# sharc-lab/FlowGNN

Measured on AMD Instinct MI355X. Metric: graphs/sec on ogbg-molhiv (GIN, dim=100), higher is better.
Workload: dtype f32; 1 GPU; GIN dim=100, batched ogbg-molhiv-shaped graphs on MI355X (BASELINE configs[1]); graphs_rank0=262144, nodes_rank0=6707949, edges_rank0=14754960, parallelism=single GPU

## Files before the change

### flowgnn_amd/csrc/dev/gin_pp_device.inc

```
constexpr int PP_ROWS = 128, PP_EDGES = 640;
constexpr int PP_PIECE = 14336, PP_PIECES = 14;
constexpr int PP_HDR_OFF = 13440;
constexpr int PP_TBL_STRIDE = 52;
constexpr int PP_TBL_BYTES = EDGE_COMBOS * PP_TBL_STRIDE * 4;
constexpr int PP_DESC_RP = PP_EDGES * 2;
constexpr int PP_DESC_PERM = PP_DESC_RP + 272;
constexpr int PP_DESC_BYTES = 1792;
constexpr int PP_SUB = 7;

__global__ __launch_bounds__(128) void gin_pp_prep_kernel(const int* __restrict__ row_ptr, const int* __restrict__ src,
                                                          const uint8_t* __restrict__ ecode, const int4* __restrict__ tiles,
                                                          uint8_t* __restrict__ desc, int n_tiles, int ntc) {
    constexpr int NKEY = 18;
    __shared__ int s_cnt[2][NKEY];
    const int tile = blockIdx.x;
    if (tile >= n_tiles) return;
    const int4 t = tiles[tile];
    const int t0 = t.x;
    int rows = t.y;
    if (rows > PP_ROWS) rows = PP_ROWS;
    const int e0 = row_ptr[t0];
    int ne = row_ptr[t0 + rows] - e0;
    if (ne > PP_EDGES) ne = PP_EDGES;
    uint8_t* d = desc + (size_t)tile * PP_DESC_BYTES;
// ... 29 lines not shown
        }
    const int pos = below + mine;
    const int kt = pos >> 4, j = pos & 15;
    if (ntc == 1) {
        d[PP_DESC_PERM + pos] = (uint8_t)r;
        return;
    }
    const int w4 = kt < 4 ? kt : 7 - kt, nt = kt < 4 ? 0 : 1;
    d[PP_DESC_PERM + w4 * 32 + nt * 16 + j] = (uint8_t)r;
}

#define PP_LD(off) (*reinterpret_cast<const uint4_t*>(wb + (off) + lane * 16))
template <bool PACKED, int NTC>
__device__ __forceinline__ void pp_w2(const char* wb, int lane, const uint4_t (&hb_hi)[NTC], const uint4_t (&hb_lo)[NTC], float4_t (&acc2)[NTC][GS_T2]) {
    if constexpr (PACKED) {
        uint4_t p[GS_T2];
#pragma unroll
        for (int t = 0; t < GS_T2; t++) p[t] = PP_LD(t * 1024);
#pragma unroll
        for (int t = 0; t < GS_T2; t++) {
            acc2[0][t] = GS_MFMA16(p[t], hb_hi[0], acc2[0][t]);
            if constexpr (NTC == 2) acc2[NTC - 1][t] = GS_MFMA16(p[t], hb_hi[NTC - 1], acc2[NTC - 1][t]);
        }
    } else {
        uint4_t f0[2], f1[2];
#define PP_U2_LOAD(F, T) F[0] = PP_LD((2 * (T)) * 1024); F[1] = PP_LD((2 * (T) + 1) * 1024);
#define PP_U2_MFMA(F, T)                                                                                    \
    acc2[0][T] = GS_MFMA16(F[0], hb_hi[0], acc2[0][T]);                                                     \
    if constexpr (NTC == 2) acc2[NTC - 1][T] = GS_MFMA16(F[0], hb_hi[NTC - 1], acc2[NTC - 1][T]);           \
    acc2[0][T] = GS_MFMA16(F[0], hb_lo[0], acc2[0][T]);                                                     \
    if constexpr (NTC == 2) acc2[NTC - 1][T] = GS_MFMA16(F[0], hb_lo[NTC - 1], acc2[NTC - 1][T]);           \
    acc2[0][T] = GS_MFMA16(F[1], hb_hi[0], acc2[0][T]);                                                     \
    if constexpr (NTC == 2) acc2[NTC - 1][T] = GS_MFMA16(F[1], hb_hi[NTC - 1], acc2[NTC - 1][T]);
        PP_U2_LOAD(f0, 0) GR_SB();
        PP_U2_LOAD(f1, 1) GR_SB(); PP_U2_MFMA(f0, 0) GR_SB();
        PP_U2_LOAD(f0, 2) GR_SB(); PP_U2_MFMA(f1, 1) GR_SB();
        PP_U2_LOAD(f1, 3) GR_SB(); PP_U2_MFMA(f0, 2) GR_SB();
        PP_U2_LOAD(f0, 4) GR_SB(); PP_U2_MFMA(f1, 3) GR_SB();
        PP_U2_LOAD(f1, 5) GR_SB(); PP_U2_MFMA(f0, 4) GR_SB();
        PP_U2_LOAD(f0, 6) GR_SB(); PP_U2_MFMA(f1, 5) GR_SB();
        PP_U2_MFMA(f0, 6) GR_SB();
#undef PP_U2_LOAD
#undef PP_U2_MFMA
    }
}

template <int NTL, bool DOT, int NTC>
__device__ __forceinline__ void pp_w1(const char* wb, int lane, int g, const uint4_t (&in_hi)[NTC][3], const uint4_t (&in_lo)[NTC][3],
                                      const uint4_t (&in_tb)[NTC], uint4_t (&hb_hi)[NTC], uint4_t (&hb_lo)[NTC], float& vmax,
                                      const float* u_step, float (&dot)[NTC]) {
    uint4_t f0[2], f1[2];
    float4_t acc1[NTC];
#define PP_U1_LOAD(F, TL, KS) F[0] = PP_LD((TL) * 6144 + (2 * (KS)) * 1024); F[1] = PP_LD((TL) * 6144 + (2 * (KS) + 1) * 1024);
#define PP_U1_MFMA1(F, KS)                                                                                  \
    acc1[0] = GS_MFMA16(F[0], in_hi[0][KS], acc1[0]);                                                       \
    if constexpr (NTC == 2) acc1[NTC - 1] = GS_MFMA16(F[0], in_hi[NTC - 1][KS], acc1[NTC - 1]);             \
    acc1[0] = GS_MFMA16(F[0], in_lo[0][KS], acc1[0]);                                                       \
    if constexpr (NTC == 2) acc1[NTC - 1] = GS_MFMA16(F[0], in_lo[NTC - 1][KS], acc1[NTC - 1]);             \
    acc1[0] = GS_MFMA16(F[1], in_hi[0][KS], acc1[0]);                                                       \
    if constexpr (NTC == 2) acc1[NTC - 1] = GS_MFMA16(F[1], in_hi[NTC - 1][KS], acc1[NTC - 1]);
#define PP_TAIL_LOAD(F, TL) F[0] = *reinterpret_cast<const uint4_t*>(wb + GRC_TAIL_OFF + (TL) * 512 + (lane & 31) * 16);
#define PP_BIAS(TL) acc1[0] = *reinterpret_cast<const float4_t*>(wb + GRC_B1_OFF + (TL) * 64 + g * 16);
#define PP_FINISH(TL)                                                                                     \
    _Pragma("unroll") for (int nt = 0; nt < NTC; nt++) {                                                    \
        float4_t r = acc1[nt];                                                                            \
        r.x = gs_relu(r.x); r.y = gs_relu(r.y); r.z = gs_relu(r.z); r.w = gs_relu(r.w);                   \
        if constexpr (DOT) {                                                                              \
            const float4 uu = *reinterpret_cast<const float4*>(u_step + 16 * (TL) + 4 * g);              \
            dot[nt] += r.x * uu.x; dot[nt] += r.y * uu.y; dot[nt] += r.z * uu.z; dot[nt] += r.w * uu.w;   \
            continue;                                                                                     \
        }                                                                                                 \
        vmax = __builtin_fmaxf(__builtin_fmaxf(vmax, r.x), r.y);                                          \
        vmax = __builtin_fmaxf(__builtin_fmaxf(vmax, r.z), r.w);                                          \
        if ((TL) == 0) { GS_SPLIT2(r.x, r.y, hb_hi[nt].x, hb_lo[nt].x); GS_SPLIT2(r.z, r.w, hb_hi[nt].y, hb_lo[nt].y); } \
        else { GS_SPLIT2(r.x, r.y, hb_hi[nt].z, hb_lo[nt].z); GS_SPLIT2(r.z, r.w, hb_hi[nt].w, hb_lo[nt].w); }           \
    }
    PP_U1_LOAD(f1, 0, 0)
    PP_BIAS(0)
    GR_SB();
    if constexpr (NTC == 2) acc1[NTC - 1] = acc1[0];
    PP_U1_LOAD(f0, 0, 1) GR_SB(); PP_U1_MFMA1(f1, 0) GR_SB();
    PP_U1_LOAD(f1, 0, 2) GR_SB(); PP_U1_MFMA1(f0, 1) GR_SB();
    PP_TAIL_LOAD(f0, 0) GR_SB(); PP_U1_MFMA1(f1, 2) GR_SB();
    if constexpr (NTL == 2) { PP_U1_LOAD(f1, 1, 0) GR_SB(); }
    acc1[0] = GS_MFMA16(f0[0], in_tb[0], acc1[0]);
    if constexpr (NTC == 2) acc1[NTC - 1] = GS_MFMA16(f0[0], in_tb[NTC - 1], acc1[NTC - 1]);
    if constexpr (NTL == 2) {
        PP_FINISH(0)
        PP_BIAS(1)
        if constexpr (NTC == 2) acc1[NTC - 1] = acc1[0];
        PP_U1_LOAD(f0, 1, 1) GR_SB(); PP_U1_MFMA1(f1, 0) GR_SB();
        PP_U1_LOAD(f1, 1, 2) GR_SB(); PP_U1_MFMA1(f0, 1) GR_SB();
        PP_TAIL_LOAD(f0, 1) GR_SB(); PP_U1_MFMA1(f1, 2) GR_SB();
        acc1[0] = GS_MFMA16(f0[0], in_tb[0], acc1[0]);
        if constexpr (NTC == 2) acc1[NTC - 1] = GS_MFMA16(f0[0], in_tb[NTC - 1], acc1[NTC - 1]);
        PP_FINISH(1)
    } else if constexpr (DOT) {
        PP_FINISH(0)
    } else {
        PP_FINISH(0)
#pragma unroll
        for (int nt = 0; nt < NTC; nt++) {
            const uint32_t ox = __shfl(hb_hi[nt].x, lane & 31, 64), oy = __shfl(hb_hi[nt].y, lane & 31, 64);
            const bool own = g < 2;
            hb_hi[nt] = own ? (uint4_t){hb_hi[nt].x, hb_hi[nt].y, hb_lo[nt].x, hb_lo[nt].y} : (uint4_t){ox, oy, 0u, 0u};
        }
    }
    asm volatile("" : "+v"(vmax));
#undef PP_U1_LOAD
#undef PP_U1_MFMA1
#undef PP_TAIL_LOAD
#undef PP_BIAS
#undef PP_FINISH
}
#undef PP_LD

__device__ __forceinline__ void pp_dma(const void* gsrc, void* ldst, int bytes, int wi, int nw, int lane) {
    const int pieces = (bytes + 1023) >> 10;
    const uint32_t lb = lds_addr_of(ldst);
    for (int pc = wi; pc < pieces; pc += nw) {
        const int left = bytes - pc * 1024;
        if (left >= 1024 || lane * 16 < left) lds_dma16(reinterpret_cast<const char*>(gsrc) + (size_t)pc * 1024, (uint32_t)lane * 16u, lb + pc * 1024);
    }
}
__device__ __forceinline__ void pp_dma_slice(const void* gsrc, void* ldst, int bytes, int first, int count, int wi, int nw, int lane) {
    const int pieces = (bytes + 1023) >> 10;
    const uint32_t lb = lds_addr_of(ldst);
    for (int pc = first + wi; pc < first + count && pc < pieces; pc += nw) {
        const int left = bytes - pc * 1024;
        if (left >= 1024 || lane * 16 < left) lds_dma16(reinterpret_cast<const char*>(gsrc) + (size_t)pc * 1024, (uint32_t)lane * 16u, lb + pc * 1024);
    }
}

// ... 340 lines not shown
```

### flowgnn_amd/csrc/gin_split.hip

```cpp
#include "gin_split.h"

#include <cmath>
#include <cstring>
#include <cstdlib>
#include <cstdio>
#include <vector>

#include "device_common.h"

#ifndef GS_SINGLE_PRODUCT
#define GS_SINGLE_PRODUCT 0
#endif
#ifndef GS_POOL_TU
#define GS_POOL_TU 0
#endif
#ifndef GS_NLOGIT_TU
#define GS_NLOGIT_TU 0
#endif
#ifndef GS_POOLSUM_TU
#define GS_POOLSUM_TU 0
#endif
#ifndef GS_POOL_MAX
#define GS_POOL_MAX 0
#endif
// ... 53 lines not shown
    } while (0)

typedef _Float16 half2_t __attribute__((ext_vector_type(2)));
__device__ __forceinline__ uint32_t gs_pack_rne(float a, float b) { return __builtin_bit_cast(uint32_t, (half2_t){(_Float16)a, (_Float16)b}); }
__device__ __forceinline__ float gs_rne(float a) { return (float)(_Float16)a; }
#define GS_OPER2(F16_, a, b, HI, LO)                                              \
    do {                                                                          \
        if constexpr (F16_) { (HI) = gs_pack_rne((a), (b)); (LO) = 0u; }          \
        else { GS_SPLIT2(a, b, HI, LO); }                                         \
    } while (0)

__device__ __forceinline__ float gs_relu(float x) {
    const int b = __builtin_bit_cast(int, x);
    return __builtin_bit_cast(float, b > 0 ? b : 0);
}

constexpr int GS_HUB = 8;
constexpr int GS_MAXHUB = 4;
template <int CTRL>
__device__ __forceinline__ float gs_dpp(float v) {
    return __builtin_bit_cast(float, __builtin_amdgcn_update_dpp(0, __builtin_bit_cast(int, v), CTRL, 0xF, 0xF, true));
}

template <int WAVES>
__device__ __forceinline__ void gs_issue_chunk(const uint8_t* __restrict__ gchunk, char* lds_buf, int wave, int lane) {
#pragma unroll
    for (int p = 0; p < (27 + WAVES - 1) / WAVES; p++) {
        const int piece = wave + WAVES * p;
        if (piece < 26 || (piece == 26 && lane < 40)) {
            const uint8_t* g = gchunk + piece * 1024 + lane * 16;
            __builtin_amdgcn_global_load_lds((const __attribute__((address_space(1))) void*)g,
                                             (__attribute__((address_space(3))) void*)(lds_buf + piece * 1024), 16, 0, 0);
        }
    }
}

template <int NT, bool F16>
__device__ __forceinline__ void gs_step(const char* wb, int s, int lane, int g, const uint4_t (&in_hi)[NT][3],
                                        const uint4_t (&in_lo)[NT][3], const float (&in_t)[NT], uint4_t (&h_hi)[NT],
                                        uint4_t (&h_lo)[NT], float4_t (&acc2)[NT][GS_T2], float& vmax) {
    uint4_t n_hi[NT], n_lo[NT];
    if (s < GS_STEPS - 1) {
        float4_t acc1[2][NT];
#pragma unroll
        for (int tl = 0; tl < 2; tl++) {
            const float4 b = *reinterpret_cast<const float4*>(wb + GS_B1_OFF + tl * 64 + g * 16);
#pragma unroll
            for (int nt = 0; nt < NT; nt++) acc1[tl][nt] = (float4_t){b.x, b.y, b.z, b.w};
        }
#pragma unroll
        for (int ks = 0; ks < 3; ks++) {
            uint4_t a[2][2];
#pragma unroll
            for (int tl = 0; tl < 2; tl++)
#pragma unroll
                for (int p = 0; p < (F16 ? 1 : 2); p++)
                    a[tl][p] = *reinterpret_cast<const uint4_t*>(wb + ((ks * 2 + tl) * 2 + p) * 1024 + lane * 16);
#pragma unroll
            for (int tl = 0; tl < 2; tl++)
#pragma unroll
                for (int nt = 0; nt < NT; nt++) acc1[tl][nt] = GS_MFMA16(a[tl][0], in_hi[nt][ks], acc1[tl][nt]);
            if constexpr (!F16) {
#pragma unroll
                for (int tl = 0; tl < 2; tl++)
#pragma unroll
                    for (int nt = 0; nt < NT; nt++) acc1[tl][nt] = GS_MFMA16(a[tl][0], in_lo[nt][ks], acc1[tl][nt]);
#pragma unroll
                for (int tl = 0; tl < 2; tl++)
#pragma unroll
                    for (int nt = 0; nt < NT; nt++) acc1[tl][nt] = GS_MFMA16(a[tl][1], in_hi[nt][ks], acc1[tl][nt]);
            }
        }
#pragma unroll
        for (int tl = 0; tl < 2; tl++) {
            const float at = *reinterpret_cast<const float*>(wb + GS_TAIL_OFF + tl * 256 + lane * 4);
#pragma unroll
            for (int nt = 0; nt < NT; nt++) acc1[tl][nt] = GS_MFMA32(at, in_t[nt], acc1[tl][nt]);
        }
#pragma unroll
        for (int nt = 0; nt < NT; nt++) {
            float4_t r0 = acc1[0][nt], r1 = acc1[1][nt];
            r0.x = gs_relu(r0.x); r0.y = gs_relu(r0.y); r0.z = gs_relu(r0.z); r0.w = gs_relu(r0.w);
            r1.x = gs_relu(r1.x); r1.y = gs_relu(r1.y); r1.z = gs_relu(r1.z); r1.w = gs_relu(r1.w);
            vmax = __builtin_fmaxf(__builtin_fmaxf(vmax, r0.x), r0.y);
            vmax = __builtin_fmaxf(__builtin_fmaxf(vmax, r0.z), r0.w);
            vmax = __builtin_fmaxf(__builtin_fmaxf(vmax, r1.x), r1.y);
            vmax = __builtin_fmaxf(__builtin_fmaxf(vmax, r1.z), r1.w);
            asm volatile("" : "+v"(vmax));
            GS_OPER2(F16, r0.x, r0.y, n_hi[nt].x, n_lo[nt].x);
            GS_OPER2(F16, r0.z, r0.w, n_hi[nt].y, n_lo[nt].y);
            GS_OPER2(F16, r1.x, r1.y, n_hi[nt].z, n_lo[nt].z);
            GS_OPER2(F16, r1.z, r1.w, n_hi[nt].w, n_lo[nt].w);
        }
    }
    if (s > 0) {
#pragma unroll
        for (int t0 = 0; t0 < GS_T2; t0 += 2) {
            uint4_t a[2][2];
#pragma unroll
            for (int tl = 0; tl < 2; tl++)
#pragma unroll
                for (int p = 0; p < (F16 ? 1 : 2); p++)
                    if (t0 + tl < GS_T2)
                        a[tl][p] = *reinterpret_cast<const uint4_t*>(wb + GS_W2_OFF + ((t0 + tl) * 2 + p) * 1024 + lane * 16);
#pragma unroll
            for (int tl = 0; tl < 2; tl++)
#pragma unroll
                for (int nt = 0; nt < NT; nt++)
                    if (t0 + tl < GS_T2) acc2[nt][t0 + tl] = GS_MFMA16(a[tl][0], h_hi[nt], acc2[nt][t0 + tl]);
            if constexpr (!F16) {
#pragma unroll
                for (int tl = 0; tl < 2; tl++)
#pragma unroll
                    for (int nt = 0; nt < NT; nt++)
                        if (t0 + tl < GS_T2) acc2[nt][t0 + tl] = GS_MFMA16(a[tl][0], h_lo[nt], acc2[nt][t0 + tl]);
#pragma unroll
                for (int tl = 0; tl < 2; tl++)
#pragma unroll
                    for (int nt = 0; nt < NT; nt++)
                        if (t0 + tl < GS_T2) acc2[nt][t0 + tl] = GS_MFMA16(a[tl][1], h_hi[nt], acc2[nt][t0 + tl]);
            }
        }
    }
    if (s < GS_STEPS - 1) {
#pragma unroll
        for (int nt = 0; nt < NT; nt++) { h_hi[nt] = n_hi[nt]; h_lo[nt] = n_lo[nt]; }
    }
}

#if GS_EPS
template <int NT, int WAVES, bool F16>
#else
template <int NT, int WAVES>
#endif
__global__ __launch_bounds__(WAVES * 64) void gin_layer_split_kernel(const float* __restrict__ h, float* __restrict__ hout,
                                                               const int* __restrict__ row_ptr,
                                                               const int* __restrict__ src,
                                                               const uint8_t* __restrict__ ecode,
                                                               const float* __restrict__ ecomb,
                                                               const uint8_t* __restrict__ wchunks, int n_tot, int relu_out,
                                                               int* __restrict__ range_flag, const float* __restrict__ pool_w
#if GS_EPS
                                                               , float self_s
// ... 231 lines not shown
                float4_t r = acc2[nt][t2] * oscale;
                if (relu_out) { r.x = gs_relu(r.x); r.y = gs_relu(r.y); r.z = gs_relu(r.z); r.w = gs_relu(r.w); }
                *reinterpret_cast<float4*>(row + col) = make_float4(r.x, r.y, r.z, r.w);
            }
        }
    }
    }
    if (__any(!(vmax < 6.0e4f))) {
        if (lane == 0) atomicOr(range_flag, 1);
    }
}

constexpr int GR_ROWS = 256;
constexpr int GR_EDGES = 1280;
constexpr float GR_MSG_SCALE = 1.0f / 65536.0f, GR_MSG_UNSCALE = 65536.0f;
constexpr int GR_WAVES = 8;
constexpr int GR_STEPS = 7;

constexpr int GRC_PK_OFF = 6144;
constexpr int GRC_PK6_OFF = 12288 + 512;
constexpr int GRC_TAIL_OFF = 12288;
constexpr int GRC_B1_OFF = 13312;
constexpr int GRC_W2_OFF = 13440;
constexpr int GRC_CHUNK_BYTES = 27776;
constexpr int GRC_CHUNK_STRIDE = 28672;

#ifndef GR_DEALERS
#define GR_DEALERS 4
#endif
#ifndef GR_DEAL_BASE
#define GR_DEAL_BASE 0
#endif
template <int DEAL>
__device__ __forceinline__ int gr_dealer(int wave) {
    if (DEAL >= GR_WAVES) return wave;
    const int d = wave - GR_DEAL_BASE;
    return (d >= 0 && d < DEAL) ? d : -1;
}
template <int DEAL = GR_DEALERS>
__device__ __forceinline__ void grc_issue_chunk(const uint8_t* __restrict__ gchunk, char* lds_buf, int wave, int lane) {
    wave = gr_dealer<DEAL>(wave);
    if (wave < 0) return;
    const uint32_t lb = lds_addr_of(lds_buf);
#pragma unroll
    for (int p = 0; p < (28 + DEAL - 1) / DEAL; p++) {
        const int piece = wave + DEAL * p;
        if (piece < 27 || (piece == 27 && lane < 8)) lds_dma16(gchunk + piece * 1024, (uint32_t)lane * 16u, lb + piece * 1024);
    }
}

template <int DEAL = GR_DEALERS>
__device__ __forceinline__ void grc_issue_chunk_w1(const uint8_t* __restrict__ gchunk, char* lds_buf, int wave, int lane) {
    wave = gr_dealer<DEAL>(wave);
    if (wave < 0) return;
    const uint32_t lb = lds_addr_of(lds_buf);
#pragma unroll
    for (int p = 0; p < (14 + DEAL - 1) / DEAL; p++) {
        const int piece = wave + DEAL * p;
        if (piece < 13 || (piece == 13 && lane < 8)) lds_dma16(gchunk + piece * 1024, (uint32_t)lane * 16u, lb + piece * 1024);
    }
}

#define GR_LD(off) (*reinterpret_cast<const uint4_t*>(wb + (off) + lane * 16))
#define GR_SB() __builtin_amdgcn_sched_barrier(0)
#ifndef GR_DEFER
#define GR_DEFER false
#endif
#ifndef GR_PRIO_HALF
#define GR_PRIO_HALF true
#endif
// ... 14 lines not shown
#define GR_PRIO_BY_PHASE true
#endif

struct GrNoHook { __device__ __forceinline__ void operator()() const {} };
template <int KIND, bool F16, bool PEND_IN = false, bool PEND_OUT = false, class HOOK = GrNoHook>
__device__ __forceinline__ void gr_step(const char* wb, int lane, int g, const uint4_t (&in_hi)[2][3], const uint4_t (&in_lo)[2][3],
                                        const uint4_t (&in_tb)[2], uint4_t (&hb_hi)[2], uint4_t (&hb_lo)[2], float4_t (&acc2)[2][GS_T2],
                                        float& vmax, float4_t (&pend)[2], const float* u_step = nullptr, float* dot = nullptr, int wave = 0,
                                        HOOK hook = HOOK()) {
    static_assert(KIND == 0 || KIND == 1 || KIND == 4 || KIND == 5, "step kinds");
    constexpr bool DO2 = KIND == 1, DO1 = true, DOT = KIND >= 4;
#define GR_PRIO_FLIP(TO_OLD) if (GR_FLIP) { if ((wave >= 4) != (TO_OLD)) __builtin_amdgcn_s_setprio(1); else __builtin_amdgcn_s_setprio(0); }
    constexpr int NTL = KIND == 5 ? 1 : 2;
    uint4_t f0[2], f1[2];
#define GR_U2_LOAD(F, T) F[0] = GR_LD(GRC_W2_OFF + (2 * (T)) * 1024); if constexpr (!F16) F[1] = GR_LD(GRC_W2_OFF + (2 * (T) + 1) * 1024);
#define GR_U2_MFMA(F, T)                                              \
    acc2[0][T] = GS_MFMA16(F[0], hb_hi[0], acc2[0][T]);               \
    acc2[1][T] = GS_MFMA16(F[0], hb_hi[1], acc2[1][T]);               \
    if constexpr (!F16) {                                             \
        acc2[0][T] = GS_MFMA16(F[0], hb_lo[0], acc2[0][T]);           \
        acc2[1][T] = GS_MFMA16(F[0], hb_lo[1], acc2[1][T]);           \
        acc2[0][T] = GS_MFMA16(F[1], hb_hi[0], acc2[0][T]);           \
        acc2[1][T] = GS_MFMA16(F[1], hb_hi[1], acc2[1][T]);           \
    }
#define GR_U1_LOAD(F, TL, KS) F[0] = GR_LD((TL) * 6144 + (2 * (KS)) * 1024); if constexpr (!F16) F[1] = GR_LD((TL) * 6144 + (2 * (KS) + 1) * 1024);
    float4_t acc1[2];
#define GR_U1_MFMA1(F, KS)                                            \
    acc1[0] = GS_MFMA16(F[0], in_hi[0][KS], acc1[0]);                 \
    acc1[1] = GS_MFMA16(F[0], in_hi[1][KS], acc1[1]);                 \
    if constexpr (!F16) {                                             \
        acc1[0] = GS_MFMA16(F[0], in_lo[0][KS], acc1[0]);             \
        acc1[1] = GS_MFMA16(F[0], in_lo[1][KS], acc1[1]);             \
        acc1[0] = GS_MFMA16(F[1], in_hi[0][KS], acc1[0]);             \
        acc1[1] = GS_MFMA16(F[1], in_hi[1][KS], acc1[1]);             \
    }
#define GR_TAIL_LOAD(F, TL) F[0] = *reinterpret_cast<const uint4_t*>(wb + GRC_TAIL_OFF + (TL) * 512 + (lane & 31) * 16);
#define GR_BIAS(TL) acc1[0] = *reinterpret_cast<const float4_t*>(wb + GRC_B1_OFF + (TL) * 64 + g * 16);
#define GR_FINISH(TL) GR_FINISH_FROM(acc1, TL)
#define GR_FINISH_FROM(SRC, TL)                                                                           \
    _Pragma("unroll") for (int nt = 0; nt < 2; nt++) {                                                    \
        float4_t r = SRC[nt];                                                                             \
        r.x = gs_relu(r.x); r.y = gs_relu(r.y); r.z = gs_relu(r.z); r.w = gs_relu(r.w);                   \
        if constexpr (DOT) {                                                                              \
            if constexpr (F16) {  \
                vmax = __builtin_fmaxf(__builtin_fmaxf(vmax, r.x), r.y);                                  \
                vmax = __builtin_fmaxf(__builtin_fmaxf(vmax, r.z), r.w);                                  \
                r.x = gs_rne(r.x); r.y = gs_rne(r.y); r.z = gs_rne(r.z); r.w = gs_rne(r.w);               \
            }                                                                                             \
            const float4 uu = *reinterpret_cast<const float4*>(u_step + 16 * (TL) + 4 * g);              \
            dot[nt] += r.x * uu.x; dot[nt] += r.y * uu.y; dot[nt] += r.z * uu.z; dot[nt] += r.w * uu.w;   \
            continue;                                                                                     \
        }                                                                                                 \
        vmax = __builtin_fmaxf(__builtin_fmaxf(vmax, r.x), r.y);                                          \
        vmax = __builtin_fmaxf(__builtin_fmaxf(vmax, r.z), r.w);                                          \
        if ((TL) == 0) { GS_OPER2(F16, r.x, r.y, hb_hi[nt].x, hb_lo[nt].x); GS_OPER2(F16, r.z, r.w, hb_hi[nt].y, hb_lo[nt].y); } \
        else { GS_OPER2(F16, r.x, r.y, hb_hi[nt].z, hb_lo[nt].z); GS_OPER2(F16, r.z, r.w, hb_hi[nt].w, hb_lo[nt].w); }           \
    }
    if constexpr (DO2) {
        GR_U2_LOAD(f0, 0)
        GR_SB();
        GR_U2_LOAD(f1, 1) GR_SB();
        if constexpr (PEND_IN) { GR_FINISH_FROM(pend, 1) GR_SB(); }
        GR_U2_MFMA(f0, 0) GR_SB();
        GR_U2_LOAD(f0, 2) GR_SB(); GR_U2_MFMA(f1, 1) GR_SB();
        GR_U2_LOAD(f1, 3) GR_SB(); GR_U2_MFMA(f0, 2) GR_SB();
        GR_U2_LOAD(f0, 4) GR_SB(); GR_U2_MFMA(f1, 3) GR_SB();
        GR_U2_LOAD(f1, 5) GR_SB(); GR_U2_MFMA(f0, 4) GR_SB();
        GR_U2_LOAD(f0, 6) GR_SB(); GR_U2_MFMA(f1, 5) GR_SB();
        GR_U1_LOAD(f1, 0, 0)
        GR_BIAS(0)
        GR_SB();
        GR_U2_MFMA(f0, 6)
        GR_SB();
        GR_PRIO_FLIP(true)
    }
    if constexpr (DO1) {
        if constexpr (!DO2) {
            GR_U1_LOAD(f1, 0, 0)
            GR_BIAS(0)
            GR_SB();
        }
        acc1[1] = acc1[0];
        GR_U1_LOAD(f0, 0, 1) GR_SB(); GR_U1_MFMA1(f1, 0) GR_SB();
        GR_U1_LOAD(f1, 0, 2) GR_SB(); GR_U1_MFMA1(f0, 1) GR_SB();
        GR_TAIL_LOAD(f0, 0) GR_SB(); GR_U1_MFMA1(f1, 2) GR_SB();
        if constexpr (NTL == 2) { GR_U1_LOAD(f1, 1, 0) GR_SB(); }
        acc1[0] = GS_MFMA16(f0[0], in_tb[0], acc1[0]);
        acc1[1] = GS_MFMA16(f0[0], in_tb[1], acc1[1]);
        if constexpr (NTL == 2) {
            if constexpr (!DO2) { GR_PRIO_FLIP(true) }
            GR_FINISH(0)
            GR_BIAS(1)
            if constexpr (DOT) { GR_SB(); hook(); GR_SB(); }
            acc1[1] = acc1[0];
            GR_U1_LOAD(f0, 1, 1) GR_SB(); GR_U1_MFMA1(f1, 0) GR_SB();
            GR_U1_LOAD(f1, 1, 2) GR_SB(); GR_U1_MFMA1(f0, 1) GR_SB();
            GR_TAIL_LOAD(f0, 1) GR_SB(); GR_U1_MFMA1(f1, 2) GR_SB();
            acc1[0] = GS_MFMA16(f0[0], in_tb[0], acc1[0]);
            acc1[1] = GS_MFMA16(f0[0], in_tb[1], acc1[1]);
            if constexpr (PEND_OUT) { pend[0] = acc1[0]; pend[1] = acc1[1]; }
            else { GR_FINISH(1) }
        } else {
            static_assert(DOT, "a one-tile step is the folded layer's last (KIND 5)");
            GR_SB(); hook(); GR_SB();
            GR_FINISH(0)
        }
        asm volatile("" : "+v"(vmax));
    }
    if constexpr (DO2 || NTL == 2) { GR_PRIO_FLIP(false) }
#undef GR_PRIO_FLIP
#undef GR_U1_MFMA1
#undef GR_TAIL_LOAD
#undef GR_BIAS
#undef GR_FINISH
#undef GR_FINISH_FROM
#undef GR_U2_LOAD
#undef GR_U2_MFMA
#undef GR_U1_LOAD
}
template <int STORE, bool F16>
__device__ __forceinline__ void gr_step_final(const char* wb, int lane, int g, const uint4_t (&in_hi)[2][3], const uint4_t (&in_lo)[2][3],
                                              const uint4_t (&in_tb)[2], const uint4_t (&hb_hi)[2], const uint4_t (&hb_lo)[2],
                                              float4_t (&acc2)[2][GS_T2], float& vmax, float oscale, float* rw0, float* rw1) {
    uint4_t f0[2], f1[2], pa, hp[2];
    float4_t acc1[2];
#define GRF_U2_LOAD(F, T) F[0] = GR_LD(GRC_W2_OFF + (2 * (T)) * 1024); if constexpr (!F16) F[1] = GR_LD(GRC_W2_OFF + (2 * (T) + 1) * 1024);
#define GRF_U2_MFMA(F, T)                                             \
    acc2[0][T] = GS_MFMA16(F[0], hb_hi[0], acc2[0][T]);               \
    acc2[1][T] = GS_MFMA16(F[0], hb_hi[1], acc2[1][T]);               \
    if constexpr (!F16) {                                             \
        acc2[0][T] = GS_MFMA16(F[0], hb_lo[0], acc2[0][T]);           \
        acc2[1][T] = GS_MFMA16(F[0], hb_lo[1], acc2[1][T]);           \
        acc2[0][T] = GS_MFMA16(F[1], hb_hi[0], acc2[0][T]);           \
        acc2[1][T] = GS_MFMA16(F[1], hb_hi[1], acc2[1][T]);           \
    }
#define GRF_U1_LOAD(F, KS) F[0] = GR_LD((2 * (KS)) * 1024); if constexpr (!F16) F[1] = GR_LD((2 * (KS) + 1) * 1024);
#define GRF_U1_MFMA(F, KS)                                            \
    acc1[0] = GS_MFMA16(F[0], in_hi[0][KS], acc1[0]);                 \
    acc1[1] = GS_MFMA16(F[0], in_hi[1][KS], acc1[1]);                 \
    if constexpr (!F16) {                                             \
        acc1[0] = GS_MFMA16(F[0], in_lo[0][KS], acc1[0]);             \
        acc1[1] = GS_MFMA16(F[0], in_lo[1][KS], acc1[1]);             \
        acc1[0] = GS_MFMA16(F[1], in_hi[0][KS], acc1[0]);             \
        acc1[1] = GS_MFMA16(F[1], in_hi[1][KS], acc1[1]);             \
    }
#define GRF_PK_LOAD(P, T)                                                                                                          \
    if constexpr ((T) < 6) P = GR_LD(GRC_PK_OFF + (T) * 1024);                                                                     \
    else P = (lane & 15) < 4 ? *reinterpret_cast<const uint4_t*>(wb + GRC_PK6_OFF + ((((lane >> 4) << 2) | (lane & 3)) << 4)) : (uint4_t){0u, 0u, 0u, 0u};
#define GRF_PK_MFMA(P, T)                                  \
    acc2[0][T] = GS_MFMA16(P, hp[0], acc2[0][T]);          \
    acc2[1][T] = GS_MFMA16(P, hp[1], acc2[1][T]);
#define GRF_STORE(T)                                                                                                  \
    if constexpr (STORE != 0) {                                                                                       \
        constexpr int col0_ = 16 * (T);                                                                               \
        if (col0_ + 4 * g < GS_D) {                                                                                   \
            float4_t r0_ = acc2[0][T] * oscale, r1_ = acc2[1][T] * oscale;                                            \
            if constexpr (STORE == 1) {                                                                               \
                r0_.x = gs_relu(r0_.x); r0_.y = gs_relu(r0_.y); r0_.z = gs_relu(r0_.z); r0_.w = gs_relu(r0_.w);       \
                r1_.x = gs_relu(r1_.x); r1_.y = gs_relu(r1_.y); r1_.z = gs_relu(r1_.z); r1_.w = gs_relu(r1_.w);       \
            }                                                                                                         \
            *reinterpret_cast<float4_t*>(rw0 + col0_ + 4 * g) = r0_;                                                  \
            *reinterpret_cast<float4_t*>(rw1 + col0_ + 4 * g) = r1_;                                                  \
        }                                                                                                             \
    }
    GRF_U1_LOAD(f1, 0)
    acc1[0] = *reinterpret_cast<const float4_t*>(wb + GRC_B1_OFF + g * 16);
    GR_SB();
    acc1[1] = acc1[0];
    GRF_U1_LOAD(f0, 1) GR_SB(); GRF_U1_MFMA(f1, 0) GR_SB();
    GRF_U1_LOAD(f1, 2) GR_SB(); GRF_U1_MFMA(f0, 1) GR_SB();
    f0[0] = *reinterpret_cast<const uint4_t*>(wb + GRC_TAIL_OFF + (lane & 31) * 16); GR_SB();
    GRF_U1_MFMA(f1, 2) GR_SB();
    GRF_U2_LOAD(f1, 0) GR_SB();
    acc1[0] = GS_MFMA16(f0[0], in_tb[0], acc1[0]);
    acc1[1] = GS_MFMA16(f0[0], in_tb[1], acc1[1]);
    GR_SB();
    GRF_U2_LOAD(f0, 1) GRF_PK_LOAD(pa, 0) GR_SB();
    GRF_U2_MFMA(f1, 0) GR_SB();
#pragma unroll
    for (int nt = 0; nt < 2; nt++) {
        float4_t r = acc1[nt];
        r.x = gs_relu(r.x); r.y = gs_relu(r.y); r.z = gs_relu(r.z); r.w = gs_relu(r.w);
        vmax = __builtin_fmaxf(__builtin_fmaxf(vmax, r.x), r.y);
        vmax = __builtin_fmaxf(__builtin_fmaxf(vmax, r.z), r.w);
        uint32_t hx, hy, lx, ly;
        GS_OPER2(F16, r.x, r.y, hx, lx);
        GS_OPER2(F16, r.z, r.w, hy, ly);
        const uint32_t ox = __shfl(hx, lane & 31, 64), oy = __shfl(hy, lane & 31, 64);
        hp[nt] = g < 2 ? (uint4_t){hx, hy, lx, ly} : (uint4_t){ox, oy, 0u, 0u};
    }
    asm volatile("" : "+v"(vmax));
    GR_SB();
    GRF_PK_MFMA(pa, 0) GR_SB();
    GRF_U2_LOAD(f1, 2) GRF_PK_LOAD(pa, 1) GR_SB(); GRF_U2_MFMA(f0, 1) GRF_PK_MFMA(pa, 1) GR_SB(); GRF_STORE(0) GR_SB();
    GRF_U2_LOAD(f0, 3) GRF_PK_LOAD(pa, 2) GR_SB(); GRF_U2_MFMA(f1, 2) GRF_PK_MFMA(pa, 2) GR_SB(); GRF_STORE(1) GR_SB();
    GRF_U2_LOAD(f1, 4) GRF_PK_LOAD(pa, 3) GR_SB(); GRF_U2_MFMA(f0, 3) GRF_PK_MFMA(pa, 3) GR_SB(); GRF_STORE(2) GR_SB();
    GRF_U2_LOAD(f0, 5) GRF_PK_LOAD(pa, 4) GR_SB(); GRF_U2_MFMA(f1, 4) GRF_PK_MFMA(pa, 4) GR_SB(); GRF_STORE(3) GR_SB();
    GRF_U2_LOAD(f1, 6) GRF_PK_LOAD(pa, 5) GR_SB(); GRF_U2_MFMA(f0, 5) GRF_PK_MFMA(pa, 5) GR_SB(); GRF_STORE(4) GR_SB();
    GRF_PK_LOAD(pa, 6) GR_SB();                    GRF_U2_MFMA(f1, 6) GRF_PK_MFMA(pa, 6) GR_SB(); GRF_STORE(5) GR_SB();
    GRF_STORE(6)
#undef GRF_U2_LOAD
#undef GRF_U2_MFMA
#undef GRF_U1_LOAD
#undef GRF_U1_MFMA
#undef GRF_PK_LOAD
#undef GRF_PK_MFMA
#undef GRF_STORE
}
#undef GR_LD

struct GrTile { int t0, rows, g0, g1; };

__device__ __forceinline__ void gr_issue_ecomb(const float* __restrict__ ecomb, char* lds_buf, int wave, int lane) {
    wave = gr_dealer<GR_DEALERS>(wave);
    if (wave < 0) return;
#pragma unroll
    for (int r = 0; r < (24 + GR_DEALERS - 1) / GR_DEALERS; r++) {
        const int piece = wave + GR_DEALERS * r;
        if (piece < 23 || (piece == 23 && lane < 28)) lds_dma16(reinterpret_cast<const char*>(ecomb) + piece * 1024, (uint32_t)lane * 16u, lds_addr_of(lds_buf) + piece * 1024);
    }
}
__device__ __forceinline__ void gr_issue_rows(const float* __restrict__ h0, char* s_rows, const GrTile& t, int part, int wave, int lane) {
    wave = gr_dealer<GR_DEALERS>(wave);
    if (wave < 0) return;
    const int np = (t.rows * (GS_D * 4) + 1023) >> 10;
// ... 943 lines not shown
    }
}


#if defined(FLOWGNN_DEV) && !GS_SINGLE_PRODUCT
#include "dev/gin_pp_device.inc"
#endif

#if !GS_SINGLE_PRODUCT
inline float pow2_scale(const float* w, size_t n) {
    float m = 0.0f;
    for (size_t i = 0; i < n; i++) m = std::fmax(m, std::fabs(w[i]));
    if (!(m > 0.0f) || !std::isfinite(m)) return 1.0f;
    return std::ldexp(1.0f, -std::ilogb(m));
}

inline void put_split(uint8_t* frag, int lane, int e, float v, bool f16 = false) {
    const _Float16 hi = (_Float16)v;
    const _Float16 lo = f16 ? (_Float16)0.0f : (_Float16)(v - (float)hi);
    std::memcpy(frag + lane * 16 + e * 2, &hi, 2);
    std::memcpy(frag + 1024 + lane * 16 + e * 2, &lo, 2);
}

#endif
}

#if !(GS_POOL_TU || GS_POOLSUM_TU || GS_NLOGIT_TU)
#define GS_LAYER_LAUNCH(NODES, WAVES, ...)                                                                                                   \
    gin_layer_split_kernel<__VA_ARGS__><<<(int)ceil_div_ll(a.n_tot, NODES), WAVES * 64, 0, s>>>(a.h, a.hout, a.row_ptr, a.src, a.ecode, a.ecomb, \
                                                                                                a.chunks, a.n_tot, a.relu_out, a.range_flag,     \
                                                                                                a.pool_w GS_LAYER_TRAILER)
#if GS_EPS_TU
#define GS_LAYER_LAUNCHER launch_gin_layer_split_eps
#define GS_LAYER_TRAILER , *a.self_s
#define GS_LAYER_SHAPE(NT, WAVES, NODES)                                  \
    do {                                                                  \
        if (a.f16) GS_LAYER_LAUNCH(NODES, WAVES, NT, WAVES, true);        \
        else GS_LAYER_LAUNCH(NODES, WAVES, NT, WAVES, false);             \
    } while (0)
#else
#if GS_SINGLE_PRODUCT
#define GS_LAYER_LAUNCHER launch_gin_layer_split_f16
#else
#define GS_LAYER_LAUNCHER launch_split_nt
#endif
#define GS_LAYER_TRAILER
// ... 63 lines not shown
#undef GR_LAUNCH_FE
#endif
#undef GR_LAUNCH
}
#undef GR_TRAILER
#undef GR_DISPATCHER

#if !GS_SINGLE_PRODUCT
void gin_split_pack_layer(const float* w1, const float* b1, const float* w2, const float* b2, uint8_t* out, bool f16) {
    std::memset(out, 0, GS_LAYER_BYTES);
    const float s1 = pow2_scale(w1, (size_t)GS_H * GS_D);
    const float s2 = pow2_scale(w2, (size_t)GS_D * GS_H);
    for (int s = 0; s < GS_STEPS; s++) {
        uint8_t* ck = out + (size_t)s * GS_CHUNK_STRIDE;
        if (s < GS_STEPS - 1) {
            for (int tl = 0; tl < 2; tl++) {
                const int t = 2 * s + tl;
                for (int lane = 0; lane < 64; lane++) {
                    const int i = lane & 15, gk = lane >> 4;
                    const int o = 16 * t + i;
                    for (int ks = 0; ks < 3; ks++)
                        for (int e = 0; e < 8; e++) {
                            const int f = 16 * (2 * ks + (e >> 2)) + 4 * gk + (e & 3);
                            put_split(ck + (size_t)((ks * 2 + tl) * 2) * 1024, lane, e, o < GS_H ? w1[o * GS_D + f] * s1 : 0.0f, f16);
                        }
                    float tail = o < GS_H ? w1[o * GS_D + 96 + gk] * s1 : 0.0f;
                    if (f16) tail = (float)(_Float16)tail;
                    std::memcpy(ck + GS_TAIL_OFF + tl * 256 + lane * 4, &tail, 4);
                }
                for (int x = 0; x < 16; x++) {
                    const int o = 16 * t + x;
                    const float b = o < GS_H ? b1[o] * s1 : 0.0f;
                    std::memcpy(ck + GS_B1_OFF + tl * 64 + x * 4, &b, 4);
                }
            }
        }
        if (s > 0) {
            const int ks = s - 1;
            for (int t2 = 0; t2 < GS_T2; t2++)
                for (int lane = 0; lane < 64; lane++) {
                    const int i = lane & 15, gk = lane >> 4;
                    const int d = 16 * t2 + i;
                    for (int e = 0; e < 8; e++) {
                        const int k = 16 * (2 * ks + (e >> 2)) + 4 * gk + (e & 3);
                        put_split(ck + GS_W2_OFF + (size_t)(t2 * 2) * 1024, lane, e, (d < GS_D && k < GS_H) ? w2[d * GS_H + k] * s2 : 0.0f, f16);
                    }
                }
        } else {
            for (int x = 0; x < 16 * GS_T2; x++) {
                const float b = x < GS_D ? b2[x] * s1 * s2 : 0.0f;
                std::memcpy(ck + GS_W2_OFF + x * 4, &b, 4);
            }
            const float os = 1.0f / (s1 * s2);
            std::memcpy(ck + GS_W2_OFF + 112 * 4, &os, 4);
        }
    }
}

size_t gin_resident_layer_bytes() { return (size_t)GS_STEPS * GRC_CHUNK_STRIDE; }

void gin_resident_head_fold(const float* w1_last, const float* w2_last, const float* b2_last, const float* pool_w, float* out, bool f16) {
    const double s1 = (double)pow2_scale(w1_last, (size_t)GS_H * GS_D);
    for (int k = 0; k < 208; k++) {
        double a = 0.0;
        if (k < GS_H)
            for (int d = 0; d < GS_D; d++) a += (double)w2_last[(size_t)d * GS_H + k] * (double)pool_w[d];
        out[k] = f16 ? (float)(_Float16)(a / s1) : (float)(a / s1);
    }
// ... 3 lines not shown
}

void gin_resident_pack_layer(const float* w1, const float* b1, const float* w2, const float* b2, uint8_t* out, bool merged, bool f16) {
    std::memset(out, 0, gin_resident_layer_bytes());
    const float s1 = pow2_scale(w1, (size_t)GS_H * GS_D);
    const float s2 = pow2_scale(w2, (size_t)GS_D * GS_H);
    auto w1s = [&](int o, int f) { return (o < GS_H && f < GS_D) ? w1[o * GS_D + f] * s1 : 0.0f; };
    auto w2s = [&](int d, int k) { return (d < GS_D && k < GS_H) ? w2[d * GS_H + k] * s2 : 0.0f; };
    auto hi16 = [](float v) { return (_Float16)v; };
    auto lo16 = [f16](float v) { const _Float16 h = (_Float16)v; return f16 ? (_Float16)0.0f : (_Float16)(v - (float)h); };
    auto put16 = [](uint8_t* p, _Float16 v) { std::memcpy(p, &v, 2); };
    for (int s = 0; s < GS_STEPS; s++) {
        uint8_t* ck = out + (size_t)s * GRC_CHUNK_STRIDE;
        if (s < GS_STEPS - 1) {
            for (int tl = 0; tl < 2; tl++) {
                const int t = 2 * s + tl;
                if (merged && t == 13) continue;
                for (int lane = 0; lane < 64; lane++) {
                    const int i = lane & 15, gk = lane >> 4;
                    const int o = 16 * t + i;
                    for (int ks = 0; ks < 3; ks++)
                        for (int e = 0; e < 8; e++) {
                            const int f = 16 * (2 * ks + (e >> 2)) + 4 * gk + (e & 3);
                            put_split(ck + (size_t)tl * 6144 + (size_t)(ks * 2) * 1024, lane, e, w1s(o, f), f16);
                        }
                    if (lane < 32) {
                        uint8_t* tp = ck + GRC_TAIL_OFF + tl * 512 + lane * 16;
                        for (int e = 0; e < 4; e++) {
                            const float v = w1s(o, 96 + e);
                            if (gk == 0) { put16(tp + e * 2, hi16(v)); put16(tp + 8 + e * 2, hi16(v)); }
                            else { put16(tp + e * 2, lo16(v)); put16(tp + 8 + e * 2, (_Float16)0.0f); }
                        }
                    }
                }
                for (int x = 0; x < 16; x++) {
                    const int o = 16 * t + x;
                    const float b = o < GS_H ? b1[o] * s1 : 0.0f;
                    std::memcpy(ck + GRC_B1_OFF + tl * 64 + x * 4, &b, 4);
                }
            }
        }
        if (s >= 1 && s <= 6) {
            const int ks = s - 1;
            for (int t2 = 0; t2 < GS_T2; t2++)
                for (int lane = 0; lane < 64; lane++) {
                    const int i = lane & 15, gk = lane >> 4;
                    const int d = 16 * t2 + i;
                    for (int e = 0; e < 8; e++) {
                        const int k = 16 * (2 * ks + (e >> 2)) + 4 * gk + (e & 3);
                        put_split(ck + GRC_W2_OFF + (size_t)(t2 * 2) * 1024, lane, e, w2s(d, k), f16);
                    }
                }
        } else if (s == 7) {
            for (int t2 = 0; t2 < GS_T2; t2++)
                for (int lane = 0; lane < 64; lane++) {
                    const int i = lane & 15, gk = lane >> 4;
                    const int d = 16 * t2 + i;
                    uint8_t* fp = ck + GRC_W2_OFF + (size_t)t2 * 1024 + lane * 16;
                    if (merged) {
                        uint8_t* c6 = out + (size_t)6 * GRC_CHUNK_STRIDE;
                        if (t2 < 6) fp = c6 + GRC_PK_OFF + (size_t)t2 * 1024 + lane * 16;
                        else if (i < 4) fp = c6 + GRC_PK6_OFF + ((gk << 2) | i) * 16;
                        else continue;
                    }
                    const int k0 = 192 + 4 * (gk & 1);
                    for (int e = 0; e < 4; e++) {
                        const float v = w2s(d, k0 + e);
                        if (gk < 2) { put16(fp + e * 2, hi16(v)); put16(fp + 8 + e * 2, hi16(v)); }
                        else { put16(fp + e * 2, lo16(v)); put16(fp + 8 + e * 2, (_Float16)0.0f); }
                    }
                }
        } else {
            for (int x = 0; x < 16 * GS_T2; x++) {
// ... 126 lines not shown
```

Measured before the change: 35.14 million graphs/s.

## Row-pack partial output tiles into single fragment with permlane fold

For the partially filled last output tiles (W1 tile 12 with 8 real rows, W2 tile 6 with 4 real rows), hi and lo split halves are packed into the unused rows of one fragment instead of two separate fragments. A permlane swap and add then folds the rows back together. This removes one fragment load and one set of MFMAs per step on those tiles and shrinks the weight chunk by one 1 KB piece for LDS DMA. In exchange it adds cross-lane permlane ops with nops, and it depends on the host-side packing layout matching the device folding exactly.

Result: no change. 35.30 million graphs/s (median of 6 runs) (+0.4%).

```diff
diff --git a/flowgnn_amd/csrc/dev/gin_pp_device.inc b/flowgnn_amd/csrc/dev/gin_pp_device.inc
--- a/flowgnn_amd/csrc/dev/gin_pp_device.inc
+++ b/flowgnn_amd/csrc/dev/gin_pp_device.inc
@@ -75,6 +75,8 @@
             acc2[0][t] = GS_MFMA16(p[t], hb_hi[0], acc2[0][t]);
             if constexpr (NTC == 2) acc2[NTC - 1][t] = GS_MFMA16(p[t], hb_hi[NTC - 1], acc2[NTC - 1][t]);
         }
+#pragma unroll
+        for (int nt = 0; nt < NTC; nt++) gs_fold_rows4(acc2[nt][GS_T2 - 1]);
     } else {
         uint4_t f0[2], f1[2];
 #define PP_U2_LOAD(F, T) F[0] = PP_LD((2 * (T)) * 1024); F[1] = PP_LD((2 * (T) + 1) * 1024);
@@ -91,8 +93,12 @@
         PP_U2_LOAD(f1, 3) GR_SB(); PP_U2_MFMA(f0, 2) GR_SB();
         PP_U2_LOAD(f0, 4) GR_SB(); PP_U2_MFMA(f1, 3) GR_SB();
         PP_U2_LOAD(f1, 5) GR_SB(); PP_U2_MFMA(f0, 4) GR_SB();
-        PP_U2_LOAD(f0, 6) GR_SB(); PP_U2_MFMA(f1, 5) GR_SB();
-        PP_U2_MFMA(f0, 6) GR_SB();
+        f0[0] = PP_LD(12 * 1024); GR_SB(); PP_U2_MFMA(f1, 5) GR_SB();
+        acc2[0][6] = GS_MFMA16(f0[0], hb_hi[0], acc2[0][6]);
+        if constexpr (NTC == 2) acc2[NTC - 1][6] = GS_MFMA16(f0[0], hb_hi[NTC - 1], acc2[NTC - 1][6]);
+        acc2[0][6] = GS_MFMA16(f0[0], hb_lo[0], acc2[0][6]);
+        if constexpr (NTC == 2) acc2[NTC - 1][6] = GS_MFMA16(f0[0], hb_lo[NTC - 1], acc2[NTC - 1][6]);
+        GR_SB();
 #undef PP_U2_LOAD
 #undef PP_U2_MFMA
     }
@@ -128,6 +134,21 @@
         if ((TL) == 0) { GS_SPLIT2(r.x, r.y, hb_hi[nt].x, hb_lo[nt].x); GS_SPLIT2(r.z, r.w, hb_hi[nt].y, hb_lo[nt].y); } \
         else { GS_SPLIT2(r.x, r.y, hb_hi[nt].z, hb_lo[nt].z); GS_SPLIT2(r.z, r.w, hb_hi[nt].w, hb_lo[nt].w); }           \
     }
+#define PP_U1P_LOAD(F, KS) F[0] = PP_LD((2 * (KS)) * 1024);
+#define PP_U1P_MFMA1(F, KS)                                                                                 \
+    acc1[0] = GS_MFMA16(F[0], in_hi[0][KS], acc1[0]);                                                       \
+    if constexpr (NTC == 2) acc1[NTC - 1] = GS_MFMA16(F[0], in_hi[NTC - 1][KS], acc1[NTC - 1]);             \
+    acc1[0] = GS_MFMA16(F[0], in_lo[0][KS], acc1[0]);                                                       \
+    if constexpr (NTC == 2) acc1[NTC - 1] = GS_MFMA16(F[0], in_lo[NTC - 1][KS], acc1[NTC - 1]);
+    if constexpr (NTL == 1 && !DOT) {
+        PP_U1P_LOAD(f1, 0)
+        PP_BIAS(0)
+        GR_SB();
+        if constexpr (NTC == 2) acc1[NTC - 1] = acc1[0];
+        PP_U1P_LOAD(f0, 1) GR_SB(); PP_U1P_MFMA1(f1, 0) GR_SB();
+        PP_U1P_LOAD(f1, 2) GR_SB(); PP_U1P_MFMA1(f0, 1) GR_SB();
+        PP_TAIL_LOAD(f0, 0) GR_SB(); PP_U1P_MFMA1(f1, 2) GR_SB();
+    } else {
     PP_U1_LOAD(f1, 0, 0)
     PP_BIAS(0)
     GR_SB();
@@ -135,6 +156,7 @@
     PP_U1_LOAD(f0, 0, 1) GR_SB(); PP_U1_MFMA1(f1, 0) GR_SB();
     PP_U1_LOAD(f1, 0, 2) GR_SB(); PP_U1_MFMA1(f0, 1) GR_SB();
     PP_TAIL_LOAD(f0, 0) GR_SB(); PP_U1_MFMA1(f1, 2) GR_SB();
+    }
     if constexpr (NTL == 2) { PP_U1_LOAD(f1, 1, 0) GR_SB(); }
     acc1[0] = GS_MFMA16(f0[0], in_tb[0], acc1[0]);
     if constexpr (NTC == 2) acc1[NTC - 1] = GS_MFMA16(f0[0], in_tb[NTC - 1], acc1[NTC - 1]);
@@ -151,6 +173,8 @@
     } else if constexpr (DOT) {
         PP_FINISH(0)
     } else {
+#pragma unroll
+        for (int nt = 0; nt < NTC; nt++) gs_fold_rows8(acc1[nt]);
         PP_FINISH(0)
 #pragma unroll
         for (int nt = 0; nt < NTC; nt++) {
@@ -162,6 +186,8 @@
     asm volatile("" : "+v"(vmax));
 #undef PP_U1_LOAD
 #undef PP_U1_MFMA1
+#undef PP_U1P_LOAD
+#undef PP_U1P_MFMA1
 #undef PP_TAIL_LOAD
 #undef PP_BIAS
 #undef PP_FINISH
diff --git a/flowgnn_amd/csrc/gin_split.hip b/flowgnn_amd/csrc/gin_split.hip
--- a/flowgnn_amd/csrc/gin_split.hip
+++ b/flowgnn_amd/csrc/gin_split.hip
@@ -99,6 +99,19 @@
     return __builtin_bit_cast(float, __builtin_amdgcn_update_dpp(0, __builtin_bit_cast(int, v), CTRL, 0xF, 0xF, true));
 }
 
+__device__ __forceinline__ float gs_fold_rows8(float v) {
+    float a = v, b = v;
+    asm volatile("s_nop 1\n\tv_permlane32_swap_b32 %0, %1\n\ts_nop 1" : "+v"(a), "+v"(b));
+    return a + b;
+}
+__device__ __forceinline__ float gs_fold_rows4(float v) {
+    float a = v, b = v;
+    asm volatile("s_nop 1\n\tv_permlane16_swap_b32 %0, %1\n\ts_nop 1" : "+v"(a), "+v"(b));
+    return a + b;
+}
+__device__ __forceinline__ void gs_fold_rows8(float4_t& a) { a.x = gs_fold_rows8(a.x); a.y = gs_fold_rows8(a.y); a.z = gs_fold_rows8(a.z); a.w = gs_fold_rows8(a.w); }
+__device__ __forceinline__ void gs_fold_rows4(float4_t& a) { a.x = gs_fold_rows4(a.x); a.y = gs_fold_rows4(a.y); a.z = gs_fold_rows4(a.z); a.w = gs_fold_rows4(a.w); }
+
 template <int WAVES>
 __device__ __forceinline__ void gs_issue_chunk(const uint8_t* __restrict__ gchunk, char* lds_buf, int wave, int lane) {
 #pragma unroll
@@ -119,6 +132,7 @@
     uint4_t n_hi[NT], n_lo[NT];
     if (s < GS_STEPS - 1) {
         float4_t acc1[2][NT];
+        const bool rowpack12 = s == GS_STEPS - 2;
 #pragma unroll
         for (int tl = 0; tl < 2; tl++) {
             const float4 b = *reinterpret_cast<const float4*>(wb + GS_B1_OFF + tl * 64 + g * 16);
@@ -144,8 +158,10 @@
                     for (int nt = 0; nt < NT; nt++) acc1[tl][nt] = GS_MFMA16(a[tl][0], in_lo[nt][ks], acc1[tl][nt]);
 #pragma unroll
                 for (int tl = 0; tl < 2; tl++)
-#pragma unroll
-                    for (int nt = 0; nt < NT; nt++) acc1[tl][nt] = GS_MFMA16(a[tl][1], in_hi[nt][ks], acc1[tl][nt]);
+                    if (tl == 1 || !rowpack12) {
+#pragma unroll
+                        for (int nt = 0; nt < NT; nt++) acc1[tl][nt] = GS_MFMA16(a[tl][1], in_hi[nt][ks], acc1[tl][nt]);
+                    }
             }
         }
 #pragma unroll
@@ -153,6 +169,12 @@
             const float at = *reinterpret_cast<const float*>(wb + GS_TAIL_OFF + tl * 256 + lane * 4);
 #pragma unroll
             for (int nt = 0; nt < NT; nt++) acc1[tl][nt] = GS_MFMA32(at, in_t[nt], acc1[tl][nt]);
+        }
+        if constexpr (!F16) {
+            if (rowpack12) {
+#pragma unroll
+                for (int nt = 0; nt < NT; nt++) gs_fold_rows8(acc1[0][nt]);
+            }
         }
 #pragma unroll
         for (int nt = 0; nt < NT; nt++) {
@@ -178,7 +200,7 @@
             for (int tl = 0; tl < 2; tl++)
 #pragma unroll
                 for (int p = 0; p < (F16 ? 1 : 2); p++)
-                    if (t0 + tl < GS_T2)
+                    if (t0 + tl < GS_T2 - p)
                         a[tl][p] = *reinterpret_cast<const uint4_t*>(wb + GS_W2_OFF + ((t0 + tl) * 2 + p) * 1024 + lane * 16);
 #pragma unroll
             for (int tl = 0; tl < 2; tl++)
@@ -195,7 +217,13 @@
                 for (int tl = 0; tl < 2; tl++)
 #pragma unroll
                     for (int nt = 0; nt < NT; nt++)
-                        if (t0 + tl < GS_T2) acc2[nt][t0 + tl] = GS_MFMA16(a[tl][1], h_hi[nt], acc2[nt][t0 + tl]);
+                        if (t0 + tl < GS_T2 - 1) acc2[nt][t0 + tl] = GS_MFMA16(a[tl][1], h_hi[nt], acc2[nt][t0 + tl]);
+            }
+        }
+        if constexpr (!F16) {
+            if (s == GS_STEPS - 1) {
+#pragma unroll
+                for (int nt = 0; nt < NT; nt++) gs_fold_rows4(acc2[nt][GS_T2 - 1]);
             }
         }
     }
@@ -473,8 +501,9 @@
 constexpr int GRC_TAIL_OFF = 12288;
 constexpr int GRC_B1_OFF = 13312;
 constexpr int GRC_W2_OFF = 13440;
-constexpr int GRC_CHUNK_BYTES = 27776;
-constexpr int GRC_CHUNK_STRIDE = 28672;
+constexpr int GRC_CHUNK_BYTES = 26752;
+constexpr int GRC_CHUNK_STRIDE = 27648;
+static_assert(GRC_CHUNK_BYTES == GRC_W2_OFF + 13 * 1024 && GRC_CHUNK_BYTES == 26 * 1024 + 128 && GRC_CHUNK_BYTES <= GRC_CHUNK_STRIDE, "GR chunk layout");
 
 #ifndef GR_DEALERS
 #define GR_DEALERS 4
@@ -494,9 +523,9 @@
     if (wave < 0) return;
     const uint32_t lb = lds_addr_of(lds_buf);
 #pragma unroll
-    for (int p = 0; p < (28 + DEAL - 1) / DEAL; p++) {
+    for (int p = 0; p < (27 + DEAL - 1) / DEAL; p++) {
         const int piece = wave + DEAL * p;
-        if (piece < 27 || (piece == 27 && lane < 8)) lds_dma16(gchunk + piece * 1024, (uint32_t)lane * 16u, lb + piece * 1024);
+        if (piece < 26 || (piece == 26 && lane < 8)) lds_dma16(gchunk + piece * 1024, (uint32_t)lane * 16u, lb + piece * 1024);
     }
 }
 
@@ -557,6 +586,14 @@
         acc2[1][T] = GS_MFMA16(F[0], hb_lo[1], acc2[1][T]);           \
         acc2[0][T] = GS_MFMA16(F[1], hb_hi[0], acc2[0][T]);           \
         acc2[1][T] = GS_MFMA16(F[1], hb_hi[1], acc2[1][T]);           \
+    }
+#define GR_U2P_LOAD(F) F[0] = GR_LD(GRC_W2_OFF + 12 * 1024);
+#define GR_U2P_MFMA(F)                                                \
+    acc2[0][6] = GS_MFMA16(F[0], hb_hi[0], acc2[0][6]);               \
+    acc2[1][6] = GS_MFMA16(F[0], hb_hi[1], acc2[1][6]);               \
+    if constexpr (!F16) {                                             \
+        acc2[0][6] = GS_MFMA16(F[0], hb_lo[0], acc2[0][6]);           \
+        acc2[1][6] = GS_MFMA16(F[0], hb_lo[1], acc2[1][6]);           \
     }
 #define GR_U1_LOAD(F, TL, KS) F[0] = GR_LD((TL) * 6144 + (2 * (KS)) * 1024); if constexpr (!F16) F[1] = GR_LD((TL) * 6144 + (2 * (KS) + 1) * 1024);
     float4_t acc1[2];
@@ -601,11 +638,11 @@
         GR_U2_LOAD(f1, 3) GR_SB(); GR_U2_MFMA(f0, 2) GR_SB();
         GR_U2_LOAD(f0, 4) GR_SB(); GR_U2_MFMA(f1, 3) GR_SB();
         GR_U2_LOAD(f1, 5) GR_SB(); GR_U2_MFMA(f0, 4) GR_SB();
-        GR_U2_LOAD(f0, 6) GR_SB(); GR_U2_MFMA(f1, 5) GR_SB();
+        GR_U2P_LOAD(f0) GR_SB(); GR_U2_MFMA(f1, 5) GR_SB();
         GR_U1_LOAD(f1, 0, 0)
         GR_BIAS(0)
         GR_SB();
-        GR_U2_MFMA(f0, 6)
+        GR_U2P_MFMA(f0)
         GR_SB();
         GR_PRIO_FLIP(true)
     }
@@ -651,6 +688,8 @@
 #undef GR_FINISH_FROM
 #undef GR_U2_LOAD
 #undef GR_U2_MFMA
+#undef GR_U2P_LOAD
+#undef GR_U2P_MFMA
 #undef GR_U1_LOAD
 }
 template <int STORE, bool F16>
@@ -669,15 +708,21 @@
         acc2[0][T] = GS_MFMA16(F[1], hb_hi[0], acc2[0][T]);           \
         acc2[1][T] = GS_MFMA16(F[1], hb_hi[1], acc2[1][T]);           \
     }
-#define GRF_U1_LOAD(F, KS) F[0] = GR_LD((2 * (KS)) * 1024); if constexpr (!F16) F[1] = GR_LD((2 * (KS) + 1) * 1024);
+#define GRF_U2P_LOAD(F) F[0] = GR_LD(GRC_W2_OFF + 12 * 1024);
+#define GRF_U2P_MFMA(F)                                               \
+    acc2[0][6] = GS_MFMA16(F[0], hb_hi[0], acc2[0][6]);               \
+    acc2[1][6] = GS_MFMA16(F[0], hb_hi[1], acc2[1][6]);               \
+    if constexpr (!F16) {                                             \
+        acc2[0][6] = GS_MFMA16(F[0], hb_lo[0], acc2[0][6]);           \
+        acc2[1][6] = GS_MFMA16(F[0], hb_lo[1], acc2[1][6]);           \
+    }
+#define GRF_U1_LOAD(F, KS) F[0] = GR_LD((2 * (KS)) * 1024);
 #define GRF_U1_MFMA(F, KS)                                            \
     acc1[0] = GS_MFMA16(F[0], in_hi[0][KS], acc1[0]);                 \
     acc1[1] = GS_MFMA16(F[0], in_hi[1][KS], acc1[1]);                 \
     if constexpr (!F16) {                                             \
         acc1[0] = GS_MFMA16(F[0], in_lo[0][KS], acc1[0]);             \
         acc1[1] = GS_MFMA16(F[0], in_lo[1][KS], acc1[1]);             \
-        acc1[0] = GS_MFMA16(F[1], in_hi[0][KS], acc1[0]);             \
-        acc1[1] = GS_MFMA16(F[1], in_hi[1][KS], acc1[1]);             \
     }
 #define GRF_PK_LOAD(P, T)                                                                                                          \
     if constexpr ((T) < 6) P = GR_LD(GRC_PK_OFF + (T) * 1024);                                                                     \
@@ -715,6 +760,7 @@
 #pragma unroll
     for (int nt = 0; nt < 2; nt++) {
         float4_t r = acc1[nt];
+        if constexpr (!F16) gs_fold_rows8(r);
         r.x = gs_relu(r.x); r.y = gs_relu(r.y); r.z = gs_relu(r.z); r.w = gs_relu(r.w);
         vmax = __builtin_fmaxf(__builtin_fmaxf(vmax, r.x), r.y);
         vmax = __builtin_fmaxf(__builtin_fmaxf(vmax, r.z), r.w);
@@ -731,11 +777,14 @@
     GRF_U2_LOAD(f0, 3) GRF_PK_LOAD(pa, 2) GR_SB(); GRF_U2_MFMA(f1, 2) GRF_PK_MFMA(pa, 2) GR_SB(); GRF_STORE(1) GR_SB();
     GRF_U2_LOAD(f1, 4) GRF_PK_LOAD(pa, 3) GR_SB(); GRF_U2_MFMA(f0, 3) GRF_PK_MFMA(pa, 3) GR_SB(); GRF_STORE(2) GR_SB();
     GRF_U2_LOAD(f0, 5) GRF_PK_LOAD(pa, 4) GR_SB(); GRF_U2_MFMA(f1, 4) GRF_PK_MFMA(pa, 4) GR_SB(); GRF_STORE(3) GR_SB();
-    GRF_U2_LOAD(f1, 6) GRF_PK_LOAD(pa, 5) GR_SB(); GRF_U2_MFMA(f0, 5) GRF_PK_MFMA(pa, 5) GR_SB(); GRF_STORE(4) GR_SB();
-    GRF_PK_LOAD(pa, 6) GR_SB();                    GRF_U2_MFMA(f1, 6) GRF_PK_MFMA(pa, 6) GR_SB(); GRF_STORE(5) GR_SB();
+    GRF_U2P_LOAD(f1) GRF_PK_LOAD(pa, 5) GR_SB();   GRF_U2_MFMA(f0, 5) GRF_PK_MFMA(pa, 5) GR_SB(); GRF_STORE(4) GR_SB();
+    GRF_PK_LOAD(pa, 6) GR_SB();                    GRF_U2P_MFMA(f1) GRF_PK_MFMA(pa, 6) GR_SB();   GRF_STORE(5) GR_SB();
+    if constexpr (!F16) { gs_fold_rows4(acc2[0][6]); gs_fold_rows4(acc2[1][6]); }
     GRF_STORE(6)
 #undef GRF_U2_LOAD
 #undef GRF_U2_MFMA
+#undef GRF_U2P_LOAD
+#undef GRF_U2P_MFMA
 #undef GRF_U1_LOAD
 #undef GRF_U1_MFMA
 #undef GRF_PK_LOAD
@@ -1725,6 +1774,14 @@
     std::memcpy(frag + 1024 + lane * 16 + e * 2, &lo, 2);
 }
 
+inline void put_rowpack(uint8_t* frag, int lane, int e, int real, float v, bool f16 = false) {
+    const int i = lane & 15;
+    const _Float16 hi = (_Float16)v;
+    const _Float16 lo = f16 ? (_Float16)0.0f : (_Float16)(v - (float)hi);
+    const _Float16 out = i < real ? hi : (i < 2 * real ? lo : (_Float16)0.0f);
+    std::memcpy(frag + lane * 16 + e * 2, &out, 2);
+}
+
 #endif
 }
 
@@ -1834,7 +1891,9 @@
                     for (int ks = 0; ks < 3; ks++)
                         for (int e = 0; e < 8; e++) {
                             const int f = 16 * (2 * ks + (e >> 2)) + 4 * gk + (e & 3);
-                            put_split(ck + (size_t)((ks * 2 + tl) * 2) * 1024, lane, e, o < GS_H ? w1[o * GS_D + f] * s1 : 0.0f, f16);
+                            uint8_t* frag = ck + (size_t)((ks * 2 + tl) * 2) * 1024;
+                            if (t == 12) put_rowpack(frag, lane, e, 8, w1[(192 + (i & 7)) * GS_D + f] * s1, f16);
+                            else put_split(frag, lane, e, o < GS_H ? w1[o * GS_D + f] * s1 : 0.0f, f16);
                         }
                     float tail = o < GS_H ? w1[o * GS_D + 96 + gk] * s1 : 0.0f;
                     if (f16) tail = (float)(_Float16)tail;
@@ -1855,7 +1914,9 @@
                     const int d = 16 * t2 + i;
                     for (int e = 0; e < 8; e++) {
                         const int k = 16 * (2 * ks + (e >> 2)) + 4 * gk + (e & 3);
-                        put_split(ck + GS_W2_OFF + (size_t)(t2 * 2) * 1024, lane, e, (d < GS_D && k < GS_H) ? w2[d * GS_H + k] * s2 : 0.0f, f16);
+                        uint8_t* frag = ck + GS_W2_OFF + (size_t)(t2 * 2) * 1024;
+                        if (t2 == GS_T2 - 1) put_rowpack(frag, lane, e, 4, k < GS_H ? w2[(96 + (i & 3)) * GS_H + k] * s2 : 0.0f, f16);
+                        else put_split(frag, lane, e, (d < GS_D && k < GS_H) ? w2[d * GS_H + k] * s2 : 0.0f, f16);
                     }
                 }
         } else {
@@ -1905,7 +1966,11 @@
                     for (int ks = 0; ks < 3; ks++)
                         for (int e = 0; e < 8; e++) {
                             const int f = 16 * (2 * ks + (e >> 2)) + 4 * gk + (e & 3);
-                            put_split(ck + (size_t)tl * 6144 + (size_t)(ks * 2) * 1024, lane, e, w1s(o, f), f16);
+                            uint8_t* frag = ck + (size_t)tl * 6144 + (size_t)(ks * 2) * 1024;
+                            if (t == 12) {
+                                put_split(frag, lane, e, w1s(o, f), f16);
+                                put_rowpack(frag, lane, e, 8, w1s(192 + (i & 7), f), f16);
+                            } else put_split(frag, lane, e, w1s(o, f), f16);
                         }
                     if (lane < 32) {
                         uint8_t* tp = ck + GRC_TAIL_OFF + tl * 512 + lane * 16;
@@ -1931,7 +1996,8 @@
                     const int d = 16 * t2 + i;
                     for (int e = 0; e < 8; e++) {
                         const int k = 16 * (2 * ks + (e >> 2)) + 4 * gk + (e & 3);
-                        put_split(ck + GRC_W2_OFF + (size_t)(t2 * 2) * 1024, lane, e, w2s(d, k), f16);
+                        if (t2 == GS_T2 - 1) put_rowpack(ck + GRC_W2_OFF + (size_t)12 * 1024, lane, e, 4, w2s(96 + (i & 3), k), f16);
+                        else put_split(ck + GRC_W2_OFF + (size_t)(t2 * 2) * 1024, lane, e, w2s(d, k), f16);
                     }
                 }
         } else if (s == 7) {
```
